# OSLL/slam-constructor

Hardware: AMD Instinct MI355X
Metric: pose-candidates*beams/sec (1080-beam scan, 2000^2 grid) (higher is better)
Workload: dtype f64; 1 GPU; cfg2: tinySLAM HC(dt 0.1, dr 0.1, failed-rounds 128), 1080 beams, 2000x2000 @0.05 m, occupancy cell; parallelism=1 gpu, ranks=1, includes_filter_and_upload=True, mode=default (canonical tree sum, device sincos; com~

## Files before the change

slam-constructor_amd/csrc/hc_resident.hip:

```cpp
#include <hip/hip_runtime.h>

#include "hc_chain_device.h"
#include "hc_resident_device.h"
#include "scan_assemble_device.h"
#include "score_device.h"

namespace slamhip {

namespace {
constexpr int kSumLanes = 256;
}

template <int H>
struct HcNextEntryT {
  double x, y, theta;
  double p[H][4];
  unsigned counts;
  unsigned flags;
};
static_assert(sizeof(HcNextEntryT<1>) == 64 && sizeof(HcNextEntryT<2>) == 96, "HcNextEntry layout");
static_assert(kHcMaxSeg + 1 <= 15, "HcNextEntry::counts: accepted rounds of a path in 4 bits");
static_assert(6 * kHcMaxInst + 6 < 4096, "HcNextEntry::counts: scorer calls of a path in 12 bits");
__device__ __forceinline__ unsigned hc_entry_counts(const HcNextCore &c, int rounds_acc) {
  return (c.failed & 0xffffu) | (((unsigned)c.batch_calls & 0xfffu) << 16) | (((unsigned)rounds_acc & 0xfu) << 28);
}

__device__ __forceinline__ void wave_min2(double &a, double &b) {
#define HCR_MIN_STEP(OFF)                              \
  {                                                    \
    const double oa = lane_xor_f64<OFF>(a), ob = lane_xor_f64<OFF>(b); \
    a = a < oa ? a : oa;                               \
    b = b < ob ? b : ob;                               \
  }
  HCR_MIN_STEP(32) HCR_MIN_STEP(16) HCR_MIN_STEP(8) HCR_MIN_STEP(4) HCR_MIN_STEP(2) HCR_MIN_STEP(1)
#undef HCR_MIN_STEP
}

constexpr int kSelRescore = -1;
constexpr int kSelFirst = -2;
constexpr int kSelStop = -3;

template <int MODEL, int NT, bool SEQ, bool BATCH, int G, bool WIN = false, bool PAIR = false, bool RAW = false>
__global__ __launch_bounds__(NT, 4) void k_hc_chain_resident(HcChainArgs a) {
  static_assert(!RAW || (!SEQ && !BATCH && !WIN && !PAIR), "RAW: the lone 1-cell chain in the default sum order only");
  constexpr int H = PAIR ? 2 : 1;
  constexpr int NTH = NT / H;
  constexpr bool CERT = !WIN;
  typedef HcNextEntryT<H> HcNextEntry;
  extern __shared__ double s_term[];
  __shared__ unsigned long long s_hash[kHcSlots + 7];
  __shared__ double s_sc[kHcSlots + 7];
  __shared__ HcInst s_mine[H][kHcShapes];
  __shared__ double s_cur[H][4];
  __shared__ int s_cur_go[H];
  __shared__ int s_sel;
  __shared__ int s_stop;
  __shared__ HcState s_st;
  __shared__ double s_part[H][4];
  __shared__ unsigned long long s_hpart[H][4];
  __shared__ double s_cert[2][16];
  __shared__ int s_cert_end;
  const long long t_kernel_begin = SLAMHIP_STAMPS_ON(a.stamps != nullptr) ? (long long)wall_clock64() : 0ll;
  const int t = threadIdx.x, wave = t >> 6;
  const int half = PAIR ? (t >= NTH ? 1 : 0) : 0;
  const int tl = t - half * NTH, lwave = tl >> 6;
  const bool init_slot = blockIdx.x + 1 == gridDim.x;
  const int slot = init_slot ? kHcSlots - 1 : (PAIR ? 2 * (int)blockIdx.x + half : (int)blockIdx.x);
  const int inst_of_slot = slot / 6, cand = slot - 6 * inst_of_slot;
  const bool exists = init_slot ? half == 0 : slot < 6 * a.max_inst;
  HcResidentCtl *const rc = a.rctl + blockIdx.y;
  HcHostOut *const host = a.host + blockIdx.y;
  const unsigned fail_epoch_at_entry = __hip_atomic_load(&rc->fail_epoch, __ATOMIC_RELAXED, __HIP_MEMORY_SCOPE_AGENT);
#ifdef SLAMHIP_TESTING
  if (a.debug_mute && (int)blockIdx.x + 1 == a.debug_mute) return;
#endif
  MapViewCP map_p;
  ScanViewCP scan_p;
  {
    const __attribute__((address_space(4))) HcChainArgs *ap0 =
        (const __attribute__((address_space(4))) HcChainArgs *)__builtin_amdgcn_kernarg_segment_ptr();
    if (BATCH) {
      const __attribute__((address_space(4))) HcJobView *jv =
          (const __attribute__((address_space(4))) HcJobView *)(unsigned long long)(a.jobs + blockIdx.y);
      map_p = &jv->map;
      scan_p = &jv->scan;
    } else {
      map_p = &ap0->map;
      scan_p = &ap0->scan;
    }
  }
  const ScanView scan = load_view(scan_p);
  const int n = scan.n;
  double br = 0.0, bc = 0.0, bs = 0.0, bw = 0.0, bf = 0.0;
  if (!RAW && tl < n) {
    br = scan.range[tl];
    bc = scan.cos_a[tl];
    bs = scan.sin_a[tl];
    bw = scan.weight[tl];
    bf = scan.factor[tl];
  }
  const bool mine_here = lwave == 1 && (t & 63) < kHcShapes && !init_slot && exists;
  constexpr int kMineQ = (int)(sizeof(HcInst) / 16);
  uint4 mine_regs[kMineQ];
  ScanPoint raw_more{0.0, 0.0, 0.0, 0.0, 0.0};
  if constexpr (RAW) {
    if (mine_here) {
      const uint4 *src = reinterpret_cast<const uint4 *>(&a.shapes[t & 63].inst[inst_of_slot]);
#pragma unroll
      for (int q = 0; q < kMineQ; ++q) mine_regs[q] = src[q];
    }
    asm volatile("" ::: "memory");
    if (tl < n) {
      const ScanPoint p = scan_assemble_point(a.raw, tl);
      br = p.range;
      bc = p.cos_a;
      bs = p.sin_a;
      bw = p.weight;
      bf = p.factor;
    }
    if (NTH + t < n) raw_more = scan_assemble_point(a.raw, NTH + t);
    asm volatile("" ::: "memory");
  }
  if (mine_here) {
    const uint4 *src = reinterpret_cast<const uint4 *>(&a.shapes[t & 63].inst[inst_of_slot]);
    uint4 *dst = reinterpret_cast<uint4 *>(&s_mine[half][t & 63]);
#pragma unroll
    for (int q = 0; q < kMineQ; ++q) dst[q] = RAW ? mine_regs[q] : src[q];
  }
  const bool ldsc = RAW || (!WIN && a.lds_consts != 0);
  const int n_more = n > NTH ? n - NTH : 0;
  double *const my_term = s_term + (PAIR ? half * a.scan.n : 0);
  double *const s_r = s_term + (PAIR ? 2 * a.scan.n : n) - NTH, *const s_ca = s_r + n_more, *const s_sa = s_ca + n_more;
  double *const s_w = s_sa + n_more, *const s_f = s_w + n_more;
  if (!RAW && ldsc) {
    for (int b = NTH + t; b < n; b += NT) {
      s_r[b] = scan.range[b];
      s_ca[b] = scan.cos_a[b];
      s_sa[b] = scan.sin_a[b];
    }
  }
  HcNextEntry *const s_tab = reinterpret_cast<HcNextEntry *>(s_term + a.tab_offset);
  if (t == 0) s_stop = fail_epoch_at_entry == a.epoch ? 1 : 0;
  if (tl < 4 && exists) {
    HcGranule *g0 = (tl & 2) ? &rc->seq[tl & 1][slot] : &rc->gran[tl & 1][slot];
    gran_store(g0, 0.0, 0ull, 0u);
  }
  const bool verify = a.verify != 0;
  const bool stamp = SLAMHIP_STAMPS_ON(a.stamps && slot == 1 && tl == 0 && blockIdx.y == 0);
  if (stamp) a.stamps[6] = t_kernel_begin;
  HcGranule *const gran = &rc->gran[0][0];
  HcGranule *const gseq = &rc->seq[0][0];
  constexpr int kGranRow = kHcSlots + 7;

  if (t == 0) {
    HcState st{};
    st.x = a.inits ? a.inits[3 * blockIdx.y] : a.init[0];
    st.y = a.inits ? a.inits[3 * blockIdx.y + 1] : a.init[1];
    st.theta = a.inits ? a.inits[3 * blockIdx.y + 2] : a.init[2];
    st.dt = a.dt0;
    st.dr = a.dr0;
    st.shape = a.shape0;
    st.first = 1;
    st.carry_cx = st.carry_cy = -1;
    st.carry_prob = -1.0;
    s_st = st;
    s_sel = kSelFirst;
    s_cert_end = 0;
  }
  __syncthreads();
  if (s_stop) return;
  if (lwave == 0) {
    const HcState &st = s_st;
    bool go = exists;
    double px = st.x, py = st.y, pth = st.theta;
    if (!init_slot && exists) {
      HcInst in;
#pragma unroll
      for (int q = 0; q < 14; ++q) in.w[q] = s_mine[half][st.shape].w[q];
      go = inst_of_slot < (int)((a.n_inst >> (8 * st.shape)) & 0xffull) &&
           (hc_is_root(in) || st.failed + hc_nfail_parent(in) < a.max_failed);
      if (go) {
        const HcRound r = hc_round_of(st, in);
        go = !(hc_trailing(r.failed, a.max_failed) && cand > 0);
        hc_candidate(r.x, r.y, r.theta, r.dt, r.dr, cand, &px, &py, &pth);
      }
    }
    double sn, cs;
    sincos(pth, &sn, &cs);
    if (tl == 0) {
      s_cur[half][0] = px;
      s_cur[half][1] = py;
      s_cur[half][2] = sn;
      s_cur[half][3] = cs;
      s_cur_go[half] = go ? 1 : 0;
    }
  }
  if constexpr (RAW) {
    for (int b = NTH + t; b < n; b += NT) {
      const ScanPoint p = b == NTH + t ? raw_more : scan_assemble_point(a.raw, b);
      s_r[b] = p.range;
      s_ca[b] = p.cos_a;
      s_sa[b] = p.sin_a;
      s_w[b] = p.weight;
      s_f[b] = p.factor;
    }
  }
  __syncthreads();

  auto write_scan_block = [&](int t, double *dst, int stride) __attribute__((always_inline)) {
    for (int q = t; q < stride; q += NT) {
      double r_ = 0.0, ca = 0.0, sa = 0.0, w = 0.0, f = 0.0;
      if (q < NT && q < n) {
        r_ = br;
        ca = bc;
        sa = bs;
        w = bw;
        f = bf;
      } else if (q < n) {
        r_ = s_r[q];
        ca = s_ca[q];
        sa = s_sa[q];
        w = s_w[q];
        f = s_f[q];
      }
      dst[q] = r_;
      dst[stride + q] = ca;
      dst[2 * stride + q] = sa;
      dst[3 * stride + q] = w;
      dst[4 * stride + q] = f;
    }
  };
  const int t_entry = t;
  for (int k = 0;; ++k) {
    const int pk = k & 1;
    int t = t_entry;
    asm volatile("" : "+v"(t));
    const int lane = t & 63;
    const int tl = PAIR ? t - half * NTH : t;
    const __attribute__((address_space(4))) HcChainArgs *ap =
        (const __attribute__((address_space(4))) HcChainArgs *)__builtin_amdgcn_kernarg_segment_ptr();
    asm volatile("" : "+s"(ap));
    MapViewCP mp = map_p;
    asm volatile("" : "+s"(mp));
    const MapView map = load_view(mp);
    if (stamp && k < 64) ap->stamps[8 * k + 0] = wall_clock64();
    const int sel = s_sel;
    if (sel == kSelStop) break;
    int go, mode = 0;
    double px, py, sn, cs;
    if (sel >= 0) {
      const HcNextEntry &e = s_tab[sel];
      const unsigned flags = e.flags;
      const bool cert_end = CERT && s_cert_end != 0;
      const int done = (int)((flags >> 3) & 1u) | (cert_end ? 1 : 0);
      go = (int)((flags >> (4 + half)) & 1u);
      px = e.p[half][0];
      py = e.p[half][1];
      sn = e.p[half][2];
      cs = e.p[half][3];
      if (wave == NT / 64 - 1 && lane < 1 + H) {
        if (lane == 0) {
          HcState &w = s_st;
          const unsigned counts = e.counts;
          const unsigned failed = counts & 0xffffu;
          const double half = hc_pow_half(failed - w.failed);
          w.x = e.x;
          w.y = e.y;
          w.theta = e.theta;
          w.dt = w.dt * half;
          w.dr = w.dr * half;
          w.recent_acc = 0.5 * w.recent_acc + (double)(counts >> 28);
          w.recent_n = 0.5 * w.recent_n + (double)((counts >> 16) & 0xfffu);
          w.failed = failed;
          w.shape = (int)(flags & 7u);
          w.done = done;
        } else {
          const int hh = lane - 1;
          s_cur[hh][0] = e.p[hh][0];
          s_cur[hh][1] = e.p[hh][1];
          s_cur[hh][2] = e.p[hh][2];
          s_cur[hh][3] = e.p[hh][3];
          s_cur_go[hh] = (int)((flags >> (4 + hh)) & 1u);
        }
      }
      long long tail_calls = 0;
      if (done && ((flags & 64u) || cert_end)) tail_calls = 6ll * (long long)(ap->max_failed - (e.counts & 0xffffu)) + 1ll;
      if (done && init_slot && tail_calls > 0 && ap->trace) {
        __syncthreads();
        HcTraceEntry *const trace = ap->trace + (size_t)blockIdx.y * (size_t)ap->trace_stride;
        const long long at0 = s_st.calls;
        const double best = s_st.best_prob, dt_e = s_st.dt, dr_e = s_st.dr;
        for (long long q = t; q < tail_calls; q += NT) {
          const double hlf = hc_pow_half((unsigned)(q / 6));
          HcTraceEntry te;
          hc_candidate(e.x, e.y, e.theta, dt_e * hlf, dr_e * hlf, (int)(q % 6), &te.x, &te.y, &te.theta);
          te.score = best;
          te.accepted = 0;
          te.pad = 0;
          if (at0 + q < ap->trace_cap) trace[at0 + q] = te;
          else host->error = 2;
        }
        __threadfence_system();
        __syncthreads();
      }
      if (done && init_slot && t == 0) {
        const HcState &w = s_st;
        const long long t_over = SLAMHIP_STAMPS_ON(ap->stamps != nullptr) ? (long long)wall_clock64() : 0ll;
        __threadfence_system();
        HcHostOut *h = host;
        h->pose[0] = e.x;
        h->pose[1] = e.y;
        h->pose[2] = e.theta;
        h->best_prob = w.best_prob;
        h->calls = w.calls + tail_calls;
        h->tail_calls = tail_calls;
        h->evaluated = w.evaluated;
        h->steps = w.steps;
        h->rescored = w.rescored;
        h->gm_cx = -1;
        h->gm_cy = -1;
        h->gm_prob = -1.0;
        __hip_atomic_store(&h->done_seq, ap->epoch, __ATOMIC_RELEASE, __HIP_MEMORY_SCOPE_SYSTEM);
        if (SLAMHIP_STAMPS_ON(ap->stamps != nullptr) && blockIdx.y == 0) {
          asm volatile("s_waitcnt vmcnt(0)" ::: "memory");
          ap->stamps[8 + 6] = t_over;
          ap->stamps[16 + 6] = wall_clock64();
        }
        if (ap->n_done) {
          __threadfence_system();
          const unsigned before = atomicAdd(ap->n_done, 1u);
          if (before + 1u == gridDim.y && ap->h_all_done)
            __hip_atomic_store(ap->h_all_done, ap->epoch, __ATOMIC_RELEASE, __HIP_MEMORY_SCOPE_SYSTEM);
        }
      }
      if constexpr (RAW) {
        if (done && init_slot && k == 1) write_scan_block(t, ap->raw.dst, (int)ap->raw.stride);
      }
      if (done) break;
    } else {
      if (sel == kSelRescore && init_slot) {
        if (wave == 0) {
          double sn_, cs_;
          sincos(s_st.theta, &sn_, &cs_);
          if (t == 0) {
            s_cur[0][0] = s_st.x;
            s_cur[0][1] = s_st.y;
            s_cur[0][2] = sn_;
            s_cur[0][3] = cs_;
            s_cur_go[0] = 1;
          }
        }
        __syncthreads();
      }
      go = s_cur_go[half];
      px = s_cur[half][0];
      py = s_cur[half][1];
      sn = s_cur[half][2];
      cs = s_cur[half][3];
      mode = sel == kSelRescore ? 1 : 0;
    }
    if (stamp && k < 64) ap->stamps[8 * k + 3] = wall_clock64();
    const unsigned tag = hc_tag(ap->tag_epoch, k);
    if (go) {
      if (WIN) {
        const double half_v = (ap->area[1] - ap->area[0]) / 2, half_h = (ap->area[3] - ap->area[2]) / 2;
        for (int b = tl; b < n; b += NTH) {
          double r_ = br, ca = bc, sa = bs, w = bw, f = bf;
          if (b != tl) {
            r_ = scan.range[b];
            ca = scan.cos_a[b];
            sa = scan.sin_a[b];
            w = scan.weight[b];
            f = scan.factor[b];
          }
          const double c = cs * ca - sn * sa;
          const double s = sn * ca + cs * sa;
          const double ox = px + r_ * c, oy = py + r_ * s;
          my_term[b] = window_probability<MODEL>(map, ap->oie, ap->oope, half_v, half_h, ox, oy) * w * f;
        }
      } else {
        constexpr int UNR = NTH == 256 ? 5 : 4;
        for (int base = tl; base < n; base += UNR * NTH) {
          double4 cell[UNR];
          double w_[UNR], f_[UNR];
  #pragma unroll
          for (int j = 0; j < UNR; ++j) {
            const int b = base + j * NTH;
            w_[j] = 0.0;
            f_[j] = 0.0;
            cell[j] = make_double4(0.0, 0.0, 0.0, 0.0);
            if ((base - lane) + j * NTH >= n) continue;
            const int bc_ = b < n ? b : n - 1;
            double r_ = br, ca = bc, sa = bs;
            w_[j] = bw;
            f_[j] = bf;
            if (j > 0 || base != tl) {
              r_ = ldsc ? s_r[bc_] : scan.range[bc_];
              ca = ldsc ? s_ca[bc_] : scan.cos_a[bc_];
              sa = ldsc ? s_sa[bc_] : scan.sin_a[bc_];
              w_[j] = RAW ? s_w[bc_] : scan.weight[bc_];
              f_[j] = RAW ? s_f[bc_] : scan.factor[bc_];
            }
            cell[j] = beam_cell<MODEL>(map, px, py, sn, cs, r_, ca, sa);
          }
  #pragma unroll
          for (int j = 0; j < UNR; ++j) {
            const int b = base + j * NTH;
            if (b < n) my_term[b] = cell_probability<MODEL>(ap->oie, cell[j]) * w_[j] * f_[j];
          }
        }
      }
    }
    double cert_t = 0.0, cert_r = 0.0;
    const bool cert_here = CERT && init_slot && half == 0 && sel >= 0 && !go && ap->inert_tail > 1;
    if (cert_here) {
      const double theta_abs = __builtin_fabs(s_tab[sel].theta);
      double tt = __builtin_inf(), tr = __builtin_inf();
      for (int b = tl; b < n; b += NTH) {
        double r_ = br, ca = bc, sa = bs;
        if (b != tl) {
          r_ = ldsc ? s_r[b] : scan.range[b];
          ca = ldsc ? s_ca[b] : scan.cos_a[b];
          sa = ldsc ? s_sa[b] : scan.sin_a[b];
        }
        double t1, t2;
        hc_cert_beam(px, py, sn, cs, theta_abs, r_, ca, sa, map.scale, map.inv_scale, &t1, &t2);
        tt = tt < t1 ? tt : t1;
        tr = tr < t2 ? tr : t2;
      }
      wave_min2(tt, tr);
      if (lane == 0) {
        s_cert[0][lwave] = tt;
        s_cert[1][lwave] = tr;
      }
    }
    __syncthreads();
    if (cert_here && tl < 64) {
      double tt = tl < NTH / 64 ? s_cert[0][tl] : __builtin_inf(), tr = tl < NTH / 64 ? s_cert[1][tl] : __builtin_inf();
      wave_min2(tt, tr);
      cert_t = tt;
      cert_r = tr;
    }
    if (stamp && k < 64) ap->stamps[8 * k + 4] = wall_clock64();
    if (go) {
      if (SEQ) {
        if (tl == 0) {
          double acc = 0.0;
          int b = 0;
          for (; b + 8 <= n; b += 8) {
            const double t0 = my_term[b], t1 = my_term[b + 1], t2 = my_term[b + 2], t3 = my_term[b + 3];
            const double t4 = my_term[b + 4], t5 = my_term[b + 5], t6 = my_term[b + 6], t7 = my_term[b + 7];
            acc = acc + t0;
            acc = acc + t1;
            acc = acc + t2;
            acc = acc + t3;
            acc = acc + t4;
            acc = acc + t5;
            acc = acc + t6;
            acc = acc + t7;
          }
          for (; b < n; ++b) acc = acc + my_term[b];
          gran_store(&gran[pk * kGranRow + slot], (scan.tot_w == 0.0) ? __builtin_nan("") : acc / scan.tot_w, 0ull, tag);
        }
      } else if (tl < kSumLanes) {
        double acc = 0.0;
        unsigned long long h = 0ull;
        unsigned k_lo = (2u * (unsigned)tl + 1u) * 0x9E3779B1u, k_hi = (2u * (unsigned)tl + 1u) * 0x85EBCA6Bu;
        for (int b = tl; b < n; b += kSumLanes) {
          const double term = my_term[b];
          acc = acc + term;
          if (verify) {
            h += term_fingerprint(term, k_lo, k_hi);
            k_lo += 2u * kSumLanes * 0x9E3779B1u;
            k_hi += 2u * kSumLanes * 0x85EBCA6Bu;
          }
        }
        wave_xor_sum_with(acc, h);
        if (lane == 0) {
          s_part[half][lwave] = acc;
          s_hpart[half][lwave] = h;
        }
      }
    }
    __syncthreads();
    if (go) {
      if (!SEQ) {
        if (tl == 0) {
          const double total = (s_part[half][0] + s_part[half][1]) + (s_part[half][2] + s_part[half][3]);
          const unsigned long long fp =
              verify ? fold_fingerprint48(s_hpart[half][0] + s_hpart[half][1] + s_hpart[half][2] + s_hpart[half][3]) : 0ull;
          gran_store(&gran[pk * kGranRow + slot], (scan.tot_w == 0.0) ? __builtin_nan("") : total / scan.tot_w, fp, tag);
        }
        if (verify && mode && tl == 64) {
          double acc = 0.0;
          for (int b = 0; b < n; ++b) acc = acc + my_term[b];
          gran_store(&gseq[pk * kGranRow + slot], (scan.tot_w == 0.0) ? __builtin_nan("") : acc / scan.tot_w, 0ull, tag);
        }
      }
      if (stamp && k < 64) ap->stamps[8 * k + 5] = wall_clock64();
    } else if (tl == 0 && exists) {
      gran_store(&gran[pk * kGranRow + slot], cert_here ? cert_t : 0.0,
                 cert_here ? (unsigned long long)__double_as_longlong(cert_r) >> 16 : 0ull, tag);
      if (verify && mode) gran_store(&gseq[pk * kGranRow + slot], 0.0, 0ull, tag);
    }
    if constexpr (RAW) {
      if (init_slot && k == 1) write_scan_block(t, ap->raw.dst, (int)ap->raw.stride);
    }

    if (wave != 0) {
      {
        const HcState &sp = s_st;
        const int shape = sp.shape;
        const int n_inst = (int)((ap->n_inst >> (8 * shape)) & 0xffull);
        const unsigned max_failed = ap->max_failed;
        for (int e = t - 64; e < 7 * n_inst; e += NT - 64) {
          const int ti = e / 7, out = e - 7 * ti;
          HcInst in;
          {
            const unsigned long long *src = &ap->shapes[shape].inst[ti].w[0];
#pragma unroll
            for (int q = 0; q < 14; ++q) in.w[q] = src[q];
          }
          if (!(hc_is_root(in) || sp.failed + hc_nfail_parent(in) < max_failed)) continue;
          const bool trailing = hc_trailing(sp.failed + hc_nfail(in), max_failed);
          if (trailing ? out > 1 : hc_child(in, out) >= 0) continue;
          const HcRound r = hc_round_of(sp, in);
          const HcNextCore c = hc_next_core(sp, in, r, out, max_failed);
          HcNextEntry &w = s_tab[e];
          w.x = c.x;
          w.y = c.y;
          w.theta = c.theta;
          w.counts = hc_entry_counts(c, hc_nseg(in) + (out > 0 ? 1 : 0));
          const bool inert = !c.done && ap->inert_tail && hc_inert(c.x, c.y, c.theta, c.dt, c.dr);
          unsigned flags = (unsigned)c.shape | (c.done || inert ? 8u : 0u) | (inert ? 64u : 0u);
#pragma unroll
          for (int hh = 0; hh < H; ++hh) {
            const int slot_h = PAIR ? 2 * (int)blockIdx.x + hh : slot;
            const int inst_h = slot_h / 6, cand_h = slot_h - 6 * inst_h;
            bool go = !c.done && !inert && !init_slot && slot_h < 6 * ap->max_inst;
            double px_ = c.x, py_ = c.y, pth_ = c.theta;
            if (go) {
              HcInst mine;
#pragma unroll
              for (int q = 0; q < 14; ++q) mine.w[q] = s_mine[hh][c.shape].w[q];
              go = inst_h < (int)((ap->n_inst >> (8 * c.shape)) & 0xffull) &&
                   (hc_is_root(mine) || c.failed + hc_nfail_parent(mine) < max_failed);
              if (go) {
                const HcRound r2 = hc_round_from(c.x, c.y, c.theta, c.dt, c.dr, c.failed, mine);
                go = !(hc_trailing(r2.failed, max_failed) && cand_h > 0);
                hc_candidate(r2.x, r2.y, r2.theta, r2.dt, r2.dr, cand_h, &px_, &py_, &pth_);
              }
            }
            double sn_ = 0.0, cs_ = 1.0;
            if (go || (CERT && init_slot && hh == 0 && ap->inert_tail > 1)) sincos(pth_, &sn_, &cs_);
            w.p[hh][0] = px_;
            w.p[hh][1] = py_;
            w.p[hh][2] = sn_;
            w.p[hh][3] = cs_;
            flags |= go ? (16u << hh) : 0u;
          }
          w.flags = flags;
        }
      }
    } else {
      const HcState &sp = s_st;
      const int n_inst = (int)((ap->n_inst >> (8 * sp.shape)) & 0xffull);
      HcInst me;
      {
        const unsigned long long *src = &ap->shapes[sp.shape].inst[lane].w[0];
#pragma unroll
        for (int q = 0; q < 14; ++q) me.w[q] = src[q];
      }
      const bool active = lane < n_inst;
      const bool reach = active && (hc_is_root(me) || sp.failed + hc_nfail_parent(me) < ap->max_failed);
      const bool trailing = reach && hc_trailing(sp.failed + hc_nfail(me), ap->max_failed);
      const int bpi = hc_bp_inst(me);
      const int bp_slot = (!active || bpi < 0) ? -1 : 6 * bpi + hc_bp_cand(me);
      const bool base_here = sp.first || sp.mode == 1;
      const int n_grid = 6 * ap->max_inst;
      const bool rescored = !SEQ && verify && sp.mode == 1;
      bool failed = false;
      {
        const HcGranule *g0 = gran + pk * kGranRow;
        unsigned spins = 0;
        for (;;) {
          u32x4 g[G];
          const HcGranule *gp[G];
          bool ok = true;
#pragma unroll
          for (int q = 0; q < G; ++q) {
            const int i = lane + 64 * q;
            gp[q] = g0 + (i < n_grid ? i : kHcSlots - 1);
          }
          gran_fetch(g, gp);
#pragma unroll
          for (int q = 0; q < G; ++q) {
            const int i = lane + 64 * q;
            const int j = i < n_grid ? i : kHcSlots - 1;
            const bool here = gran_tag(g[q]) == tag;
            ok = ok && here;
            if (here) {
              s_sc[j] = gran_score(g[q]);
              s_hash[j] = gran_hash(g[q]);
            }
          }
          if (__all(ok)) break;
          ++spins;
          if (BATCH) __builtin_amdgcn_s_sleep(8);
          if ((spins & 31u) == 0u) {
            const bool gone = __hip_atomic_load(&rc->fail_epoch, __ATOMIC_RELAXED, __HIP_MEMORY_SCOPE_AGENT) == ap->epoch;
            if (gone || spins > ap->spin_limit) {
              failed = true;
              break;
            }
          }
        }
      }
      if (stamp && k < 64) ap->stamps[8 * k + 1] = wall_clock64();
      if (failed || k + 1 >= kHcResidentMaxSteps) {
        if (lane == 0) {
          __hip_atomic_store(&rc->fail_epoch, ap->epoch, __ATOMIC_RELAXED, __HIP_MEMORY_SCOPE_AGENT);
          __hip_atomic_store(&host->error, failed ? 4 : 5, __ATOMIC_RELAXED, __HIP_MEMORY_SCOPE_SYSTEM);
          __threadfence_system();
          __hip_atomic_store(&host->done_seq, ap->epoch, __ATOMIC_RELEASE, __HIP_MEMORY_SCOPE_SYSTEM);
          s_sel = kSelStop;
        }
      } else {
        double root_prob = sp.first ? s_sc[kHcSlots - 1] : sp.best_prob;
        double s6[6];
#pragma unroll
        for (int c = 0; c < 6; ++c) s6[c] = s_sc[6 * lane + c];
        const double enter = bp_slot < 0 ? root_prob : s_sc[bp_slot];
        double run = enter;
        int out = 0;
        unsigned accmask = 0u;
        bool ambiguous = false;
        unsigned long long run_hash = 0ull;
        if (!SEQ && verify) {
          const unsigned long long root_hash = base_here ? s_hash[kHcSlots - 1] : sp.best_hash;
          unsigned long long hb = bp_slot < 0 ? root_hash : s_hash[bp_slot];
          unsigned long long h6[6];
#pragma unroll
          for (int c = 0; c < 6; ++c) h6[c] = s_hash[6 * lane + c];
          if (!rescored) {
            int amb = 0;
#pragma unroll
            for (int c = 0; c < 6; ++c) {
              const double s = s6[c];
              const double diff = __builtin_fabs(s - run);
              const double as = __builtin_fabs(s), ab = __builtin_fabs(run);
              const int live = (c == 0) | (int)!trailing;
              const int close = (int)(diff <= (as > ab ? as : ab) * 9.094947017729282e-13);
              amb |= live & close & ((int)(h6[c] != hb) | (int)(__double_as_longlong(s) != __double_as_longlong(run)));
              const bool acc = (live & (int)(run < s)) != 0;
              run = acc ? s : run;
              hb = acc ? h6[c] : hb;
              out = acc ? c + 1 : out;
              accmask |= acc ? 1u << c : 0u;
            }
            ambiguous = amb != 0;
          } else {
            const HcGranule *q0 = gseq + pk * kGranRow;
            double bdec = 0.0;
#pragma unroll 1
            for (int c = -1; c < 6; ++c) {
              const int j = c < 0 ? (bp_slot < 0 ? kHcSlots - 1 : bp_slot) : (active ? 6 * lane + c : kHcSlots - 1);
              double sd = 0.0;
              for (unsigned spins = 0;; ++spins) {
                u32x4 g[1];
                const HcGranule *gp[1] = {q0 + j};
                gran_fetch(g, gp);
                sd = gran_score(g[0]);
                if (__all(gran_tag(g[0]) == tag) || spins > ap->spin_limit) break;
              }
              if (c < 0) {
                bdec = sd;
                continue;
              }
              const bool acc = active && (c == 0 || !trailing) && bdec < sd;
              bdec = acc ? sd : bdec;
              run = acc ? s_sc[6 * lane + c] : run;
              hb = acc ? s_hash[6 * lane + c] : hb;
              out = acc ? c + 1 : out;
              accmask |= acc ? 1u << c : 0u;
            }
          }
          run_hash = hb;
        } else {
#pragma unroll
          for (int c = 0; c < 6; ++c)
            if ((c == 0 || !trailing) && run < s6[c]) {
              run = s6[c];
              out = c + 1;
              accmask |= 1u << c;
            }
        }
        bool valid = reach;
#pragma unroll
        for (int o = 0; o < 7; ++o) {
          const unsigned long long has = __ballot(reach && out == o);
          valid = valid && (me.w[o] & ~has) == 0ull;
        }
        const bool terminal = valid && (trailing || hc_child(me, out) < 0);
        const unsigned long long tmask = __ballot(terminal);
        const int tl = tmask ? __ffsll((long long)tmask) - 1 : 0;
        if (stamp && k < 64) ap->stamps[8 * k + 7] = wall_clock64();
        const bool dirty = !SEQ && verify && sp.mode == 0 && __ballot(valid && ambiguous) != 0ull;
        const int out_t = bcast_i(out, tl);
        const double run_t = bcast(run, tl);
        const int depth_t = bcast_i(hc_depth(me), tl);
        const bool trailing_t = bcast_i(trailing ? 1 : 0, tl) != 0;
        const unsigned long long run_hash_t = (unsigned long long)bcast_ll((long long)run_hash, tl);
        if (init_slot && ap->trace && !dirty) {
          HcTraceEntry *const trace = ap->trace + (size_t)blockIdx.y * (size_t)ap->trace_stride;
          const long long base = sp.calls + (sp.first ? 1 : 0);
          if (sp.first && lane == 0 && ap->trace_cap > 0) {
            HcTraceEntry e{sp.x, sp.y, sp.theta, root_prob, 1, 0};
            trace[0] = e;
          }
          if (valid) {
            const HcRound rr = hc_round_of(sp, me);
            const int nc = trailing ? 1 : 6;
            for (int c = 0; c < nc; ++c) {
              HcTraceEntry e;
              hc_candidate(rr.x, rr.y, rr.theta, rr.dt, rr.dr, c, &e.x, &e.y, &e.theta);
              e.score = s_sc[6 * lane + c];
              e.accepted = (accmask >> c) & 1u;
              e.pad = 0;
              const long long at = base + 6ll * hc_depth(me) + c;
              if (at < ap->trace_cap) trace[at] = e;
              else host->error = 2;
            }
          }
        }
        bool cert_end = false;
        if (CERT && ap->inert_tail > 1 && !sp.first && sp.mode == 0 && !dirty && tmask != 0ull) {
          const int nseg_t = bcast_i(hc_nseg(me), tl), nfail_t = bcast_i((int)hc_nfail(me), tl);
          const unsigned failed_next = sp.failed + (unsigned)nfail_t + 1u;
          if (nseg_t == 0 && out_t == 0 && !trailing_t && failed_next < ap->max_failed) {
            const double hlf = hc_pow_half((unsigned)nfail_t + 1u);
            const double t_t = s_sc[kHcSlots - 1];
            const double t_r = __longlong_as_double((long long)(s_hash[kHcSlots - 1] << 16));
            cert_end = sp.dt * hlf < t_t && sp.dr * hlf < t_r;
          }
        }
        if (stamp && k < 64) ap->stamps[8 * k + 2] = wall_clock64();
        if (lane == 0) {
          s_cert_end = cert_end ? 1 : 0;
          HcState &w = s_st;
          if (tmask == 0ull) {
            if (init_slot) {
              __hip_atomic_store(&host->error, 1, __ATOMIC_RELAXED, __HIP_MEMORY_SCOPE_SYSTEM);
              __threadfence_system();
              __hip_atomic_store(&host->done_seq, ap->epoch, __ATOMIC_RELEASE, __HIP_MEMORY_SCOPE_SYSTEM);
            }
            s_sel = kSelStop;
          } else if (!dirty) {
            w.best_prob = run_t;
            w.calls = sp.calls + (sp.first ? 1 : 0) + 6ll * depth_t + (trailing_t ? 1 : 6);
            w.evaluated = sp.evaluated + 6ll * n_inst + (sp.first ? 1 : 0);
            w.first = 0;
            w.mode = 0;
            w.steps = sp.steps + 1;
            if (!SEQ && verify) w.best_hash = run_hash_t;
            s_sel = 7 * tl + out_t;
          } else {
            w.mode = 1;
            w.steps = sp.steps + 1;
            w.evaluated = sp.evaluated + 6ll * n_inst + 1;
            w.rescored = sp.rescored + 1;
            s_sel = kSelRescore;
          }
        }
      }
    }
    __syncthreads();
  }
}

size_t hc_resident_tab_offset(int nt, int n_beams, int lds_consts, bool pair) {
  const size_t n = (size_t)(n_beams > 0 ? n_beams : 1);
  const size_t nth = (size_t)(pair ? nt / 2 : nt);
  const size_t more = lds_consts && n > nth ? n - nth : 0;
  return (pair ? 2 : 1) * n + (lds_consts > 1 ? 5 : 3) * more;
}
size_t hc_resident_lds_bytes(int nt, int n_beams, int lds_consts, int max_inst, bool pair) {
  return sizeof(double) * hc_resident_tab_offset(nt, n_beams, lds_consts, pair) +
         (pair ? sizeof(HcNextEntryT<2>) : sizeof(HcNextEntryT<1>)) * 7 * (size_t)max_inst;
}

typedef void (*HcResidentKernel)(HcChainArgs);
static HcResidentKernel hc_resident_kernel(int cell_model, const HcResidentKey &key) {
  int nt_v = 0, g_v = 0;
  if (!hc_resident_variant(key, &nt_v, &g_v)) return nullptr;
  return pick_cell_model(cell_model, [&](auto model) -> HcResidentKernel {
    constexpr int M = decltype(model)::value;
    return pick_hc_nt(nt_v, [&](auto nt) -> HcResidentKernel {
      constexpr int NT = decltype(nt)::value;
      if (key.window) return k_hc_chain_resident<M, NT, false, false, 4, true>;
      const auto sweep = [&](auto g) -> HcResidentKernel {
        constexpr int G = decltype(g)::value;
        if constexpr (NT == 512)
          if (key.batch && key.pair) return k_hc_chain_resident<M, 512, false, true, G, false, true>;
        if (key.batch) return k_hc_chain_resident<M, NT, false, true, G>;
        if constexpr (G == 4)
          if (key.raw) return k_hc_chain_resident<M, NT, false, false, 4, false, false, true>;
        if (key.raw) return nullptr;
        return key.seq ? k_hc_chain_resident<M, NT, true, false, G> : k_hc_chain_resident<M, NT, false, false, G>;
      };
      if (g_v == 2) return sweep(int_c<2>{});
      if (g_v == 4) return sweep(int_c<4>{});
      if constexpr (NT != 1024) return sweep(int_c<7>{});
      return nullptr;
    });
  });
}

static HcResidentKey key_of(const HcChainArgs &a, int nt) {
  return {nt, a.max_inst, a.seq != 0, a.jobs != nullptr, a.pair != 0, a.oope != SLAMHIP_OOPE_OBSTACLE,
          a.raw.h_range != nullptr};
}

hipError_t launch_hc_chain_resident(const HcChainArgs &a_in, int cell_model, int nt, hipStream_t stream, hipEvent_t e0,
                                    hipEvent_t e1, int n_chains) {
  if (!a_in.rctl) return hipErrorInvalidValue;
  HcChainArgs a = a_in;
  const HcResidentKey key = key_of(a, nt);
  const bool pair = key.batch && key.pair;
  const int ldsc = key.window ? 0 : (key.raw ? 2 : (a.lds_consts != 0 ? 1 : 0));
  if (key.raw && a.raw.n != a.scan.n) return hipErrorInvalidValue;
  const int grid = pair ? 3 * a.max_inst + 1 : 6 * a.max_inst + 1;
  a.tab_offset = (int)hc_resident_tab_offset(nt, a.scan.n, ldsc, pair);
  return launch_kernel(hc_resident_kernel(cell_model, key), dim3(grid, n_chains), dim3(hc_nt_of(nt)),
                       hc_resident_lds_bytes(nt, a.scan.n, ldsc, a.max_inst, pair), stream, e0, e1, a);
}

hipError_t hc_resident_capacity(int cell_model, HcResidentKey key, int n_beams, bool lds_consts, int *out_wgs,
                                int *out_per_cu) {
  key.seq = false;
  return resident_capacity_of((const void *)hc_resident_kernel(cell_model, key), key.nt,
                              hc_resident_lds_bytes(key.nt, n_beams, key.raw ? 2 : (lds_consts ? 1 : 0), key.max_inst,
                                                    key.batch && key.pair),
                              2048 / key.nt , 6, out_wgs, out_per_cu);
}

}
```

slam-constructor_amd/csrc/scan_assemble_device.h:

```cpp
#pragma once

#include <hip/hip_runtime.h>

#include "slamhip_internal.h"

namespace slamhip {

struct ScanPoint {
  double range, cos_a, sin_a, weight, factor;
};

__device__ __forceinline__ ScanPoint scan_assemble_point(const ScanAssembleArgs &a, int q) {
  ScanPoint p;
  p.range = a.h_range[q];
  const int i = a.h_kept ? a.h_kept[q] : q;
  p.cos_a = a.tab_cos[i];
  p.sin_a = a.tab_sin[i];
  p.weight = a.h_weight ? a.h_weight[q] : (a.tab_viny ? a.tab_viny[i] * sqrt(p.range) : a.w_even);
  p.factor = a.h_factor ? a.h_factor[q] : 1.0;
  return p;
}

}
```

Baseline: 13.41 billion pose-candidates*beams/s.

## Batch raw scan assembly loads in flight and defer stop check in RAW path

In the RAW scan path, the per-beam global loads (range, kept index, weight, factor, cos/sin tables) are now issued through inline-asm staged loads, two beams at a time, with a single vmcnt wait. The instance record is held in named registers and read once from constant address space, and the fail-epoch stop check is moved after the scan load, so the block's startup global-memory latency can overlap. The aim is to cut the serialized load latency in kernel prologue. In exchange it depends on hand-written asm wait ordering and now rejects multi-chain or inits launches in RAW mode.

```diff
diff --git a/slam-constructor_amd/csrc/hc_resident.hip b/slam-constructor_amd/csrc/hc_resident.hip
--- a/slam-constructor_amd/csrc/hc_resident.hip
+++ b/slam-constructor_amd/csrc/hc_resident.hip
@@ -101,31 +101,38 @@
   }
   const bool mine_here = lwave == 1 && (t & 63) < kHcShapes && !init_slot && exists;
   constexpr int kMineQ = (int)(sizeof(HcInst) / 16);
-  uint4 mine_regs[kMineQ];
-  ScanPoint raw_more{0.0, 0.0, 0.0, 0.0, 0.0};
+  static_assert(!RAW || kMineQ == 8, "RAW: the instance record in eight named registers");
+  u32x4 mine0, mine1, mine2, mine3, mine4, mine5, mine6, mine7;
+  ScanInFlight raw_first{0.0, 0.0, 0.0, 0.0, 1.0, 0}, raw_more{0.0, 0.0, 0.0, 0.0, 1.0, 0};
+  HcInst first_in = {};
+  const int n_last = n > 0 ? n - 1 : 0;
+  const bool raw_more_wave = RAW && __builtin_amdgcn_readfirstlane(NTH + (t & ~63)) < n;
   if constexpr (RAW) {
     if (mine_here) {
-      const uint4 *src = reinterpret_cast<const uint4 *>(&a.shapes[t & 63].inst[inst_of_slot]);
-#pragma unroll
-      for (int q = 0; q < kMineQ; ++q) mine_regs[q] = src[q];
+      const u32x4 *src = reinterpret_cast<const u32x4 *>(&a.shapes[t & 63].inst[inst_of_slot]);
+      mine0 = src[0];
+      mine1 = src[1];
+      mine2 = src[2];
+      mine3 = src[3];
+      mine4 = src[4];
+      mine5 = src[5];
+      mine6 = src[6];
+      mine7 = src[7];
     }
     asm volatile("" ::: "memory");
-    if (tl < n) {
-      const ScanPoint p = scan_assemble_point(a.raw, tl);
-      br = p.range;
-      bc = p.cos_a;
-      bs = p.sin_a;
-      bw = p.weight;
-      bf = p.factor;
-    }
-    if (NTH + t < n) raw_more = scan_assemble_point(a.raw, NTH + t);
-    asm volatile("" ::: "memory");
-  }
-  if (mine_here) {
+    scan_assemble_issue(a.raw, tl < n ? tl : n_last, raw_first);
+    if (raw_more_wave) scan_assemble_issue(a.raw, NTH + t < n ? NTH + t : n_last, raw_more);
+    {
+      const __attribute__((address_space(4))) HcInst *ip = (const __attribute__((address_space(4))) HcInst *)(
+          unsigned long long)&a.shapes[a.shape0].inst[init_slot ? 0 : inst_of_slot];
+#pragma unroll
+      for (int q = 0; q < 14; ++q) first_in.w[q] = ip->w[q];
+    }
+  } else if (mine_here) {
     const uint4 *src = reinterpret_cast<const uint4 *>(&a.shapes[t & 63].inst[inst_of_slot]);
     uint4 *dst = reinterpret_cast<uint4 *>(&s_mine[half][t & 63]);
 #pragma unroll
-    for (int q = 0; q < kMineQ; ++q) dst[q] = RAW ? mine_regs[q] : src[q];
+    for (int q = 0; q < kMineQ; ++q) dst[q] = src[q];
   }
   const bool ldsc = RAW || (!WIN && a.lds_consts != 0);
   const int n_more = n > NTH ? n - NTH : 0;
@@ -140,7 +147,7 @@
     }
   }
   HcNextEntry *const s_tab = reinterpret_cast<HcNextEntry *>(s_term + a.tab_offset);
-  if (t == 0) s_stop = fail_epoch_at_entry == a.epoch ? 1 : 0;
+  if (!RAW && t == 0) s_stop = fail_epoch_at_entry == a.epoch ? 1 : 0;
   if (tl < 4 && exists) {
     HcGranule *g0 = (tl & 2) ? &rc->seq[tl & 1][slot] : &rc->gran[tl & 1][slot];
     gran_store(g0, 0.0, 0ull, 0u);
@@ -154,9 +161,10 @@
 
   if (t == 0) {
     HcState st{};
-    st.x = a.inits ? a.inits[3 * blockIdx.y] : a.init[0];
-    st.y = a.inits ? a.inits[3 * blockIdx.y + 1] : a.init[1];
-    st.theta = a.inits ? a.inits[3 * blockIdx.y + 2] : a.init[2];
+    const double *const inits = RAW ? nullptr : a.inits;
+    st.x = inits ? inits[3 * blockIdx.y] : a.init[0];
+    st.y = inits ? inits[3 * blockIdx.y + 1] : a.init[1];
+    st.theta = inits ? inits[3 * blockIdx.y + 2] : a.init[2];
     st.dt = a.dt0;
     st.dr = a.dr0;
     st.shape = a.shape0;
@@ -168,7 +176,7 @@
     s_cert_end = 0;
   }
   __syncthreads();
-  if (s_stop) return;
+  if (!RAW && s_stop) return;
   if (lwave == 0) {
     const HcState &st = s_st;
     bool go = exists;
@@ -176,7 +184,7 @@
     if (!init_slot && exists) {
       HcInst in;
 #pragma unroll
-      for (int q = 0; q < 14; ++q) in.w[q] = s_mine[half][st.shape].w[q];
+      for (int q = 0; q < 14; ++q) in.w[q] = RAW ? first_in.w[q] : s_mine[half][st.shape].w[q];
       go = inst_of_slot < (int)((a.n_inst >> (8 * st.shape)) & 0xffull) &&
            (hc_is_root(in) || st.failed + hc_nfail_parent(in) < a.max_failed);
       if (go) {
@@ -196,16 +204,53 @@
     }
   }
   if constexpr (RAW) {
-    for (int b = NTH + t; b < n; b += NT) {
-      const ScanPoint p = b == NTH + t ? raw_more : scan_assemble_point(a.raw, b);
+    const auto keep = [&](int b, const ScanPoint &p) __attribute__((always_inline)) {
       s_r[b] = p.range;
       s_ca[b] = p.cos_a;
       s_sa[b] = p.sin_a;
       s_w[b] = p.weight;
       s_f[b] = p.factor;
+    };
+    scan_assemble_wait(raw_first, raw_more);
+    asm volatile("" ::"v"(mine0), "v"(mine1), "v"(mine2), "v"(mine3), "v"(mine4), "v"(mine5), "v"(mine6), "v"(mine7),
+                 "v"(fail_epoch_at_entry));
+    {
+      ScanPoint p, pm;
+      scan_assemble_finish(a.raw, raw_first, raw_more, p, pm);
+      if (tl < n) {
+        br = p.range;
+        bc = p.cos_a;
+        bs = p.sin_a;
+        bw = p.weight;
+        bf = p.factor;
+      }
+      if (NTH + t < n) keep(NTH + t, pm);
+    }
+    if (mine_here) {
+      u32x4 *dst = reinterpret_cast<u32x4 *>(&s_mine[half][t & 63]);
+      dst[0] = mine0;
+      dst[1] = mine1;
+      dst[2] = mine2;
+      dst[3] = mine3;
+      dst[4] = mine4;
+      dst[5] = mine5;
+      dst[6] = mine6;
+      dst[7] = mine7;
+    }
+    if (t == 0) s_stop = fail_epoch_at_entry == a.epoch ? 1 : 0;
+    for (int b = NTH + NT + t; b - (t & 63) < n; b += 2 * NT) {
+      ScanInFlight f0{0.0, 0.0, 0.0, 0.0, 1.0, 0}, f1{0.0, 0.0, 0.0, 0.0, 1.0, 0};
+      scan_assemble_issue(a.raw, b < n ? b : n_last, f0);
+      scan_assemble_issue(a.raw, b + NT < n ? b + NT : n_last, f1);
+      scan_assemble_wait(f0, f1);
+      ScanPoint p0, p1;
+      scan_assemble_finish(a.raw, f0, f1, p0, p1);
+      if (b < n) keep(b, p0);
+      if (b + NT < n) keep(b + NT, p1);
     }
   }
   __syncthreads();
+  if (RAW && s_stop) return;
 
   auto write_scan_block = [&](int t, double *dst, int stride) __attribute__((always_inline)) {
     for (int q = t; q < stride; q += NT) {
@@ -828,7 +873,7 @@
   const HcResidentKey key = key_of(a, nt);
   const bool pair = key.batch && key.pair;
   const int ldsc = key.window ? 0 : (key.raw ? 2 : (a.lds_consts != 0 ? 1 : 0));
-  if (key.raw && a.raw.n != a.scan.n) return hipErrorInvalidValue;
+  if (key.raw && (a.raw.n != a.scan.n || a.inits || n_chains != 1)) return hipErrorInvalidValue;
   const int grid = pair ? 3 * a.max_inst + 1 : 6 * a.max_inst + 1;
   a.tab_offset = (int)hc_resident_tab_offset(nt, a.scan.n, ldsc, pair);
   return launch_kernel(hc_resident_kernel(cell_model, key), dim3(grid, n_chains), dim3(hc_nt_of(nt)),
diff --git a/slam-constructor_amd/csrc/scan_assemble_device.h b/slam-constructor_amd/csrc/scan_assemble_device.h
--- a/slam-constructor_amd/csrc/scan_assemble_device.h
+++ b/slam-constructor_amd/csrc/scan_assemble_device.h
@@ -10,15 +10,76 @@
   double range, cos_a, sin_a, weight, factor;
 };
 
-__device__ __forceinline__ ScanPoint scan_assemble_point(const ScanAssembleArgs &a, int q) {
+__device__ __forceinline__ ScanPoint scan_point_of(const ScanAssembleArgs &a, double range, double cos_a, double sin_a,
+                                                   double viny, double h_weight, double h_factor) {
   ScanPoint p;
-  p.range = a.h_range[q];
-  const int i = a.h_kept ? a.h_kept[q] : q;
-  p.cos_a = a.tab_cos[i];
-  p.sin_a = a.tab_sin[i];
-  p.weight = a.h_weight ? a.h_weight[q] : (a.tab_viny ? a.tab_viny[i] * sqrt(p.range) : a.w_even);
-  p.factor = a.h_factor ? a.h_factor[q] : 1.0;
+  p.range = range;
+  p.cos_a = cos_a;
+  p.sin_a = sin_a;
+  p.weight = a.h_weight ? h_weight : (a.tab_viny ? viny * sqrt(p.range) : a.w_even);
+  p.factor = a.h_factor ? h_factor : 1.0;
   return p;
 }
 
+__device__ __forceinline__ ScanPoint scan_assemble_point(const ScanAssembleArgs &a, int q) {
+  const double range = a.h_range[q];
+  const int i = a.h_kept ? a.h_kept[q] : q;
+  const double cos_a = a.tab_cos[i], sin_a = a.tab_sin[i];
+  const double h_weight = a.h_weight ? a.h_weight[q] : 0.0;
+  const double viny = !a.h_weight && a.tab_viny ? a.tab_viny[i] : 0.0;
+  const double h_factor = a.h_factor ? a.h_factor[q] : 1.0;
+  return scan_point_of(a, range, cos_a, sin_a, viny, h_weight, h_factor);
 }
+
+struct ScanInFlight {
+  double range, cos_a, sin_a;
+  double wv;
+  double h_factor;
+  int kept;
+};
+__device__ __forceinline__ void staged_load(double &dst, const double *p) {
+  asm volatile("global_load_dwordx2 %0, %1, off" : "+v"(dst) : "v"(p));
+}
+__device__ __forceinline__ void staged_load(int &dst, const int *p) {
+  asm volatile("global_load_dword %0, %1, off" : "+v"(dst) : "v"(p));
+}
+__device__ __forceinline__ void scan_assemble_issue(const ScanAssembleArgs &a, int q, ScanInFlight &s) {
+  s.range = s.cos_a = s.sin_a = s.wv = 0.0;
+  s.h_factor = 1.0;
+  s.kept = q;
+  staged_load(s.range, a.h_range + q);
+  if (a.h_kept) staged_load(s.kept, a.h_kept + q);
+  if (a.h_weight) staged_load(s.wv, a.h_weight + q);
+  if (a.h_factor) staged_load(s.h_factor, a.h_factor + q);
+  if (!a.h_kept) {
+    staged_load(s.cos_a, a.tab_cos + q);
+    staged_load(s.sin_a, a.tab_sin + q);
+    if (!a.h_weight && a.tab_viny) staged_load(s.wv, a.tab_viny + q);
+  }
+}
+__device__ __forceinline__ void scan_assemble_wait(ScanInFlight &s, ScanInFlight &u) {
+  asm volatile("s_waitcnt vmcnt(0)"
+               : "+v"(s.range), "+v"(s.cos_a), "+v"(s.sin_a), "+v"(s.wv), "+v"(s.h_factor), "+v"(s.kept), "+v"(u.range),
+                 "+v"(u.cos_a), "+v"(u.sin_a), "+v"(u.wv), "+v"(u.h_factor), "+v"(u.kept)
+               :
+               : "memory");
+}
+__device__ __forceinline__ void scan_assemble_finish(const ScanAssembleArgs &a, const ScanInFlight &s,
+                                                     const ScanInFlight &u, ScanPoint &ps, ScanPoint &pu) {
+  double cs = s.cos_a, ss = s.sin_a, vs = s.wv, cu = u.cos_a, su = u.sin_a, vu = u.wv;
+  if (a.h_kept) {
+    cs = a.tab_cos[s.kept];
+    cu = a.tab_cos[u.kept];
+    ss = a.tab_sin[s.kept];
+    su = a.tab_sin[u.kept];
+    if (!a.h_weight && a.tab_viny) {
+      vs = a.tab_viny[s.kept];
+      vu = a.tab_viny[u.kept];
+    }
+    asm volatile("" ::"v"(cs), "v"(ss), "v"(vs), "v"(cu), "v"(su), "v"(vu));
+  }
+  ps = scan_point_of(a, s.range, cs, ss, vs, s.wv, s.h_factor);
+  pu = scan_point_of(a, u.range, cu, su, vu, u.wv, u.h_factor);
+}
+
+}
```

Measured after the change: 13.87 billion pose-candidates*beams/s (median of 6 runs). +3.4%, better.
